# EEA-sensors/parallel-gps

Measured on AMD Instinct MI355X. Metric: timesteps/sec (filter+smooth+log-lik), higher is better.
Workload: dtype f64; 1 GPU; c2: matern32 state-dim 2, N=2^20 steps per GPU (1048576 total), f64, irregular times, prior-sampled observations; steps_per_gpu=1048576, steps_total=1048576, state_dim=2, parallelism=1 GPU

## Files before the change

### parallel-gps_amd/csrc/pgps_ctx.hip

```cpp
#include <cstdio>
#include <new>

#include "pgps_host.h"

using namespace pgps;

namespace pgps {
int ensure(pgps_ctx* ctx, DevBuf& b, size_t bytes) {
    if (&b == &ctx->ws) ++ctx->ws_epoch;
    if (bytes <= b.cap) return PGPS_OK;
    if (b.p) HIPCHK(ctx, hipFree(b.p));
    b.p = nullptr;
    b.cap = 0;
    size_t want = bytes + bytes / 8 + 256;
    hipError_t e = hipMalloc(&b.p, want);
    if (e != hipSuccess) {
        ctx->hip_err = std::string("hipMalloc: ") + hipGetErrorString(e);
        (void)hipGetLastError();
        b.p = nullptr;
        return PGPS_E_NOMEM;
    }
    b.cap = want;
    return PGPS_OK;
}
}

extern "C" int pgps_version(void) { return 100; }

extern "C" const char* pgps_strerror(int code) {
    switch (code) {
        case PGPS_OK: return "ok";
        case PGPS_E_INVALID: return "invalid argument";
        case PGPS_E_UNSUPPORTED_DIM: return "state dimension not supported by the compiled kernels";
        case PGPS_E_HIP: return "HIP runtime error";
        case PGPS_E_NOMEM: return "out of memory";
        case PGPS_E_NUMERIC: return "non-finite result";
        case PGPS_E_NO_DEVICE: return "no HIP device";
        case PGPS_E_COMM: return "RCCL communicator error (pgps_last_hip_error)";
        default: return "unknown error";
    }
}

extern "C" int pgps_device_count(int* n) {
    if (!n) return PGPS_E_INVALID;
    int c = 0;
    if (hipGetDeviceCount(&c) != hipSuccess) c = 0;
    *n = c;
    return PGPS_OK;
}

extern "C" int pgps_create(int device, pgps_ctx** out) {
    if (!out) return PGPS_E_INVALID;
    *out = nullptr;
    int c = 0;
    if (hipGetDeviceCount(&c) != hipSuccess || c <= 0) return PGPS_E_NO_DEVICE;
    if (device < 0 || device >= c) return PGPS_E_INVALID;
    pgps_ctx* ctx = new (std::nothrow) pgps_ctx();
    if (!ctx) return PGPS_E_NOMEM;
    ctx->device = device;
    if (hipSetDevice(device) != hipSuccess ||
        hipStreamCreateWithFlags(&ctx->own_stream, hipStreamNonBlocking) != hipSuccess) {
        delete ctx;
        return PGPS_E_HIP;
    }
    ctx->stream = ctx->own_stream;
    if (hipDeviceGetAttribute(&ctx->n_cu, hipDeviceAttributeMultiprocessorCount, device) != hipSuccess) ctx->n_cu = 0;
    if (const char* e = std::getenv("PGPS_WC_ROWS2")) ctx->wc_rows2 = std::atoi(e) & 15;
    if (const char* e = std::getenv("PGPS_WC_SERIAL3")) ctx->wc_serial3 = (e[0] == '1');
    if (hipMalloc((void**)&ctx->status_word, pgps::kStatusBytes) != hipSuccess ||
        hipMemset(ctx->status_word, 0, pgps::kStatusBytes) != hipSuccess) {
        (void)hipStreamDestroy(ctx->own_stream);
        delete ctx;
        return PGPS_E_NOMEM;
    }
    *out = ctx;
    return PGPS_OK;
}

extern "C" int pgps_destroy(pgps_ctx* ctx) {
    if (!ctx) return PGPS_OK;
    (void)hipSetDevice(ctx->device);
    (void)hipStreamSynchronize(ctx->stream);
    if (ctx->comm) (void)pgps_comm_destroy(ctx);
    if (ctx->comm_buf.p) (void)hipFree(ctx->comm_buf.p);
    if (ctx->ws.p) (void)hipFree(ctx->ws.p);
    if (ctx->stamps.p) (void)hipFree(ctx->stamps.p);
    if (ctx->res_stamps.p) (void)hipFree(ctx->res_stamps.p);
    if (ctx->gadj.p) (void)hipFree(ctx->gadj.p);
    if (ctx->pin_d.p) (void)hipFree(ctx->pin_d.p);
    if (ctx->pin_h) (void)hipHostFree(ctx->pin_h);
    if (ctx->out_h) (void)hipHostFree(ctx->out_h);
    if (ctx->status_word) (void)hipFree(ctx->status_word);
    for (auto& b : ctx->st)
        if (b.p) (void)hipFree(b.p);
    for (auto& b : ctx->lti)
        if (b.p) (void)hipFree(b.p);
    for (auto& b : ctx->wide)
        if (b.p) (void)hipFree(b.p);
    if (ctx->smp.p) (void)hipFree(ctx->smp.p);
    if (ctx->smp_wide.p) (void)hipFree(ctx->smp_wide.p);
    if (ctx->probe_host) (void)hipHostFree(ctx->probe_host);
    for (auto& e : ctx->ev_pool) { (void)hipEventDestroy(e.a); (void)hipEventDestroy(e.b); }
    if (ctx->own_stream) (void)hipStreamDestroy(ctx->own_stream);
    delete ctx;
    return PGPS_OK;
}

extern "C" int pgps_set_stream(pgps_ctx* ctx, void* s) {
    if (!ctx) return PGPS_E_INVALID;
    ctx->stream = (hipStream_t)s;
    return PGPS_OK;
}

extern "C" int pgps_use_own_stream(pgps_ctx* ctx) {
    if (!ctx) return PGPS_E_INVALID;
    ctx->stream = ctx->own_stream;
    return PGPS_OK;
}

extern "C" int pgps_synchronize(pgps_ctx* ctx) {
    if (!ctx) return PGPS_E_INVALID;
    HIPCHK(ctx, hipStreamSynchronize(ctx->stream));
    return PGPS_OK;
}

extern "C" int pgps_set_chunk(pgps_ctx* ctx, int c) {
    if (!ctx || c < 0) return PGPS_E_INVALID;
    ctx->chunk = c;
    return PGPS_OK;
}

extern "C" int pgps_debug_read_stamps(pgps_ctx* ctx, long long* out, long n_values) {
    if (!ctx || !out) return PGPS_E_INVALID;
    if (!ctx->stamps.p || (size_t)n_values * sizeof(long long) > ctx->stamps.cap) return PGPS_E_INVALID;
    HIPCHK(ctx, hipStreamSynchronize(ctx->stream));
    HIPCHK(ctx, hipMemcpy(out, ctx->stamps.p, (size_t)n_values * sizeof(long long), hipMemcpyDeviceToHost));
    return PGPS_OK;
}

extern "C" int pgps_status(pgps_ctx* ctx, int* flags) {
    if (!ctx || !flags) return PGPS_E_INVALID;
    *flags = 0;
    if (!ctx->status_word) return PGPS_OK;
    HIPCHK(ctx, hipStreamSynchronize(ctx->stream));
    HIPCHK(ctx, hipMemcpy(flags, ctx->status_word, sizeof(int), hipMemcpyDeviceToHost));
// ... 372 lines not shown
```

### parallel-gps_amd/csrc/pgps_internal.h

```cpp
#pragma once

#include <hip/hip_runtime.h>
#include <hip/hip_ext.h>

#include <string>
#include <vector>

#include "../../include/pgps.h"
#include "pgps_dyn.h"

struct DevBuf {
    void* p = nullptr;
    size_t cap = 0;
};

struct pgps_ctx {
    int device = 0;
    int n_cu = 0;
    hipStream_t own_stream = nullptr;
    hipStream_t stream = nullptr;
    int chunk = 0;
    int stage_g = -1;
    int single_pass = -1;
    int lookback_window = 256;
    int block = 0;
    size_t batch_scratch = 0;
    int batch_form = 0;
    int one_launch = -1;
    long grad_pack = -1;
    int rc_scan = -1;
    int dma = -1;
    int shortcut = 1;
    int resident = -1;
    unsigned res_epoch = 0;
    DevBuf res_stamps;
    int res_stamp_blocks = 0;
    int res_delay_tile = -1;
    int res_delay_phase = 0;
    long long res_delay_ticks = 0;
    int family = 0;
    std::string hip_err;
    DevBuf ws;
    DevBuf st[12];
    bool wc_attr_done[2][17] = {};
    int wc_rows2 = 15;
    int wc_serial3 = 0;
    DevBuf lti[12];
    DevBuf stamps;
    int* status_word = nullptr;
    int host_flags = 0;
    int f32_policy = 0;
    int* probe_host = nullptr;
    int* probe_dev = nullptr;
    int probe_seq = 0;
    int f32_last_promoted = 0;
    char* pin_h = nullptr;
    DevBuf pin_d;
    char* out_h = nullptr;
    size_t out_cap = 0;
    DevBuf gadj;
    DevBuf wide[9];
    DevBuf smp;
    DevBuf smp_wide;
    DevBuf cov[6];
    DevBuf cov_wide;
    void* comm = nullptr;
    int comm_rank = 0, comm_nranks = 0;
    DevBuf comm_buf;
    struct SegTag { int phase = 0; long N = 0; int d = 0, rank = 0, nranks = 0, chunk = 0, block = 0, family = 0, stage_g = 0, dma = 0, rc_scan = 0; unsigned long epoch = 0; } seg_tag;
    unsigned long ws_epoch = 0;
    unsigned profiling = 0;
    int prof_every = 1;
    long prof_seen[PGPS_K_COUNT] = {0};
    struct EvPair { hipEvent_t a, b; int slot; };
    std::vector<EvPair> ev_pool;
    size_t ev_used = 0;
    double prof_ms[PGPS_K_COUNT] = {0};
    long prof_n[PGPS_K_COUNT] = {0};
};

struct RoctxRange {
    explicit RoctxRange(const char* name) { pgps::dyn::range_push(name); }
    ~RoctxRange() { pgps::dyn::range_pop(); }
    RoctxRange(const RoctxRange&) = delete;
    RoctxRange& operator=(const RoctxRange&) = delete;
};

// ... 57 lines not shown
    int nt;
    int* ticket;
    int* flags;
    int ll_in_apply;
    T* incl;
    int win;
    long long* stamps;
    int shortcut;
    int dform;
};

inline int seg_rec_f_len(int d) { return d * d + d + d * (d + 1) + d + 2 * d * d; }
inline int seg_rec_s_pad(int d) { int n = d * d + d + d * (d + 1) / 2; return n + (n & 1); }
inline int seg_rec_s_len(int d) { return seg_rec_s_pad(d) + 2; }

template <typename... KArgs, typename... Args>
inline void timed_launch(pgps_ctx* ctx, int slot, void (*kernel)(KArgs...), dim3 grid, dim3 block, unsigned shmem,
                         Args... args) {
    pgps_ctx::EvPair* ev = prof_acquire(ctx, slot);
    if (ev) hipExtLaunchKernelGGL(kernel, grid, block, shmem, ctx->stream, ev->a, ev->b, 0, KArgs(args)...);
    else hipLaunchKernelGGL(kernel, grid, block, shmem, ctx->stream, KArgs(args)...);
}

template <typename T>
struct GpModel {
    double lam;
    double N1[9];
    double N2[9];
    double Pinf[9];
    T H[3];
    const T* ts;
    T t_prev;
};

template <typename T>
struct GpArgs {
    ScanArgs<T> s;
    GpModel<T> m;
    const int* qslot;
    T* pmean;
    T* pvar;
};

template <typename T, int D>
int launch_gp(pgps_ctx* ctx, GpArgs<T> g, int want_filtered, int want_smoothed);

template <typename T>
struct ResArgs {
    ScanArgs<T> s;
    GpModel<T> m;
    int* bar;
    int* bar2;
    int* bar_next;
    int* flags1;
    int* flags2;
    int epoch;
    long long* stamps;
    int delay_tile;
    int delay_phase;
    long long delay_ticks;
    long long* wstamps;
};
constexpr int kResLc = 16;
constexpr int kStatusBytes = 8192;
constexpr int kResBarWord = 512;
constexpr int kResBarSet = 2 * 8 * 32;
constexpr int kResFlagWord = 1536;
constexpr int kResMaxBlocks = 256;
static_assert(kResBarWord + 2 * kResBarSet <= kResFlagWord, "barrier counters overlap the hand-off flags");
static_assert((kResFlagWord + 2 * kResMaxBlocks) * 4 <= kStatusBytes, "hand-off flags outside the status buffer");
bool resident_fits(const pgps_ctx* ctx, long N, int d, bool f32);
template <typename T, int D>
int launch_resident(pgps_ctx* ctx, ResArgs<T> ra, bool fused, bool smooth);
template <typename T, int D>
int launch_gp_adj(pgps_ctx* ctx, GpArgs<double> g, double* out);

template <typename T>
struct GpBatchArgs {
    long N;
    int Lc, nblocks;
    long nlanes;
    const T* ts;
    const T* ys;
    T t_prev;
    const double* models;
    T* spine;
    T* lpre;
    double* llpart;
    double* ll;
    T* fms;
    T* fPs;
    long bs_fm, bs_fP;
    T* sspine;
    T* lsuf;
    const int* qslot;
    T* pmean;
    T* pvar;
    long K;
};
constexpr int kGpModelStride = 32;

template <typename T, int D>
int launch_gp_batch(pgps_ctx* ctx, int B, GpBatchArgs<T> b);
template <typename T, int D>
int launch_gp_predict_batch(pgps_ctx* ctx, int B, GpBatchArgs<T> b);
template <typename T, int D>
int launch_gp_adj_batch(pgps_ctx* ctx, int B, GpBatchArgs<double> b, double* out);
constexpr size_t kBatchScratchDefault = 64u << 20;
constexpr long kBatchOneMax = 65536;

template <typename T>
int launch_merge(pgps_ctx* ctx, long N, long K, const T* ts, const T* ys, const T* tq, T* ts_m, T* ys_m, int* qslot);

int launch_grad(pgps_ctx* ctx, long N, int d, int np, const double* model, const double* ts, double t0,
                const double* ys, double* out_dev);

template <int D>
int launch_gradb(pgps_ctx* ctx, long N, int nblk, const int* bsize, int np, const double* model, const double* ts, double t0,
                 const double* ys, double* out_dev);

enum Mode { MODE_PKF, MODE_PKS, MODE_PKFS, MODE_SEG_REDUCE, MODE_SEG_FILTER, MODE_SEG_SMOOTHER };

template <typename T>
// ... 138 lines not shown
```

### parallel-gps_amd/csrc/pgps_res_inst.hip

```cpp
#include "pgps_resident.hip.h"

#ifndef PGPS_RES_T
#error "compile with -DPGPS_RES_T=<float|double> -DPGPS_RES_D=<d>"
#endif

namespace pgps {

template <typename T, int D>
int launch_resident(pgps_ctx* ctx, ResArgs<T> ra, bool fused, bool smooth) {
    HIPCHK(ctx, hipSetDevice(ctx->device));
    ScanArgs<T>& a = ra.s;
    const int max_blocks = ctx->n_cu < kResMaxBlocks ? ctx->n_cu : kResMaxBlocks;
    int lc = kResLc;
    if (ctx->resident > 0 && (ctx->chunk == 8 || ctx->chunk == 16)) lc = ctx->chunk;
    else if (a.N <= (long)kBlock * 8 * max_blocks) lc = 8;
    a.Lc = lc;
    a.nblocks = (int)((a.N + (long)kBlock * lc - 1) / ((long)kBlock * lc));
    if (a.nblocks < 1 || a.nblocks > max_blocks) return PGPS_E_INVALID;
    a.nlanes = (long)a.nblocks * kBlock;
    a.seg_first = 1;
    a.seg_last = 1;
    a.shortcut = ctx->shortcut != 0 ? 1 : 0;
    auto up = [](size_t x) { return (x + 255) / 256 * 256; };
    const size_t nb = (size_t)a.nblocks;
    size_t off = 0;
    const size_t o_spine = off;  off = up(off + nb * Dim<D>::NFILT * sizeof(T));
    const size_t o_sspine = off; off = up(off + nb * Dim<D>::NSMTH * sizeof(T));
    const size_t o_ll = off;     off = up(off + nb * sizeof(double));
    int rc = ensure(ctx, ctx->ws, off);
    if (rc) return rc;
    ctx->ws_epoch++;
    char* base = (char*)ctx->ws.p;
    a.spine = (T*)(base + o_spine);
    a.sspine = (T*)(base + o_sspine);
    a.llpart = (double*)(base + o_ll);
    a.status = ctx->status_word;
    const unsigned e = ctx->res_epoch++;
    ra.bar = ctx->status_word + kResBarWord + (e & 1u) * kResBarSet;
    ra.bar2 = ra.bar + kResBarSet / 2;
    ra.bar_next = ctx->status_word + kResBarWord + ((e + 1u) & 1u) * kResBarSet;
    ra.flags1 = ctx->status_word + kResFlagWord;
    ra.flags2 = ctx->status_word + kResFlagWord + kResMaxBlocks;
    ra.epoch = (int)(e % 0x7ffffffeu) + 1;
    ra.stamps = nullptr;
    ra.wstamps = nullptr;
    ra.delay_tile = -1;
    ra.delay_phase = 0;
    ra.delay_ticks = 0;
    const bool skew = ctx->res_delay_tile >= 0;
    if (ctx->resident == 2 || skew) {
        rc = ensure(ctx, ctx->res_stamps, nb * (16 + 8) * sizeof(long long));
        if (rc) return rc;
        if (ctx->resident == 2) ra.stamps = (long long*)ctx->res_stamps.p;
        ctx->res_stamp_blocks = a.nblocks;
    }
    if (skew) {
        HIPCHK(ctx, hipMemsetAsync(ctx->res_stamps.p, 0, nb * 16 * sizeof(long long), ctx->stream));
        HIPCHK(ctx, hipMemsetAsync(base, 0xFF, off, ctx->stream));
        ra.wstamps = (long long*)ctx->res_stamps.p;
        ra.delay_tile = ctx->res_delay_tile;
        ra.delay_phase = ctx->res_delay_phase;
        ra.delay_ticks = ctx->res_delay_ticks;
    }
    const dim3 grid(a.nblocks), block(kBlock);
    auto go = [&](auto lcv, auto fusedv, auto smoothv) {
        constexpr int L = decltype(lcv)::value;
        constexpr bool FU = decltype(fusedv)::value, SM = decltype(smoothv)::value;
        if (skew) timed_launch(ctx, PGPS_K_RESIDENT, k_pkfs_resident<T, D, L, FU, SM, true>, grid, block, 0, ra);
        else timed_launch(ctx, PGPS_K_RESIDENT, k_pkfs_resident<T, D, L, FU, SM, false>, grid, block, 0, ra);
    };
    auto pick = [&](auto lcv) {
        if (fused) { if (smooth) go(lcv, std::true_type{}, std::true_type{}); else go(lcv, std::true_type{}, std::false_type{}); }
        else { if (smooth) go(lcv, std::false_type{}, std::true_type{}); else go(lcv, std::false_type{}, std::false_type{}); }
    };
    if (lc == 8) pick(std::integral_constant<int, 8>{}); else pick(std::integral_constant<int, kResLc>{});
    HIPCHK(ctx, hipGetLastError());
    return PGPS_OK;
}

template int launch_resident<PGPS_RES_T, PGPS_RES_D>(pgps_ctx*, ResArgs<PGPS_RES_T>, bool, bool);

}
```

### parallel-gps_amd/csrc/pgps_resident.hip.h

```cpp
#pragma once

#include <type_traits>

#include "pgps_fused.hip.h"
#include "pgps_kernels.hip.h"

namespace pgps {


template <typename T, int D, int LC>
struct ResCfg {
    static constexpr int W = (int)sizeof(T), MAT = D * D, G = 4;
    static_assert(LC % G == 0, "whole sub-tiles");
    static constexpr int S = LC / G;
    using GF = StageGeom<MAT * W, G>;
    using GM = StageGeom<D * W, G>;
    static constexpr int SLOT = LC * MAT * W + 16;
    static constexpr int SLOTS = kWave * SLOT;
    static constexpr int MST = GM::BYTES > 5120 ? GM::BYTES : 5120;
    static constexpr int NSCAN = kWaves * Dim<D>::NFILT * W;
    static constexpr int BYTES = kWaves * (SLOTS + MST) + NSCAN + kWaves * 8;
};

__device__ __forceinline__ void res_wave_sync() {
    __builtin_amdgcn_fence(__ATOMIC_RELEASE, "wavefront");
    __builtin_amdgcn_wave_barrier();
    __builtin_amdgcn_fence(__ATOMIC_ACQUIRE, "wavefront");
}

template <typename T> struct ResForget;
template <> struct ResForget<double> { static constexpr double kA = 0x1p-120; };
template <> struct ResForget<float> { static constexpr float kA = 0x1p-60f; };

#define PGPS_RSTAMP(IDX)                                                                              \
    do {                                                                                              \
        if (ra.stamps && threadIdx.x == 0) ra.stamps[(long)blockIdx.x * 16 + (IDX)] = __builtin_readcyclecounter(); \
    } while (0)
#define PGPS_RSTAMP_WAVE(K)                                                                           \
    do {                                                                                              \
        if (ra.stamps && lane == 0)                                                                   \
            ra.stamps[(long)gridDim.x * 16 + (long)blockIdx.x * 8 + (K) * kWaves + wave] = __builtin_readcyclecounter(); \
    } while (0)

template <typename T>
__device__ __forceinline__ void res_skew(const ResArgs<T>& ra, int tile, int phase) {
    if (tile == ra.delay_tile && phase == ra.delay_phase) {
        const long long t0 = wall_clock64();
        ra.wstamps[(long)tile * 16 + 12] = t0;
        ra.wstamps[(long)tile * 16 + 13] = ra.delay_ticks;
        while (wall_clock64() - t0 < ra.delay_ticks) __builtin_amdgcn_s_sleep(8);
    }
}
template <typename T>
__device__ __forceinline__ void res_wstamp(const ResArgs<T>& ra, int tile, int slot) {
    if (ra.wstamps) ra.wstamps[(long)tile * 16 + slot] = wall_clock64();
}

template <typename T, int D>
__device__ __forceinline__ V4 res_pad_piece(int kind, int pos_in_rec) {
    constexpr int PER = 16 / (int)sizeof(T);
    T tmp[PER];
#pragma unroll
    for (int j = 0; j < PER; ++j) {
        const int e = (pos_in_rec * PER + j) % (D * D);
        tmp[j] = (kind == 0 && (e / D) == (e % D)) ? T(1) : T(0);
    }
    V4 v;
    __builtin_memcpy(&v, tmp, 16);
    return v;
}

template <typename T, int D, typename GEO, int PITCH>
__device__ __forceinline__ void res_issue(const char* __restrict__ g , int sb, long lim, bool full, int kind, V4* r) {
// ... 34 lines not shown
#pragma unroll
        for (int v = 0; v < NV; ++v)
            if (v >= v0 && v < v0 + nv) x[v] = *reinterpret_cast<const V4*>(base + sb * GEO::SEG + v * OPI * SLOT);
#pragma unroll
        for (int v = 0; v < NV; ++v)
            if (v >= v0 && v < v0 + nv) *reinterpret_cast<V4*>(g + ((long)sb * GEO::SEG + (long)v * OPI * PITCH) + loff) = x[v];
    } else {
#pragma unroll
        for (int v = 0; v < NV; ++v) {
            if (v < v0 || v >= v0 + nv) continue;
            const V4 x = *reinterpret_cast<const V4*>(base + sb * GEO::SEG + v * OPI * SLOT);
            if ((int)loff < lim - (sb * GEO::SEG + v * OPI * PITCH))
                *reinterpret_cast<V4*>(g + ((long)sb * GEO::SEG + (long)v * OPI * PITCH) + loff) = x;
        }
    }
}
template <typename GEO, int SLOT, int PITCH>
__device__ __forceinline__ void res_drain(char* __restrict__ g , int sb, int lim, bool full, const char* slots) {
    res_drain_part<GEO, SLOT, PITCH>(g, sb, 0, GEO::NV, lim, full, slots);
}
template <typename GEO, int PITCH>
__device__ __forceinline__ void res_drain_m(char* __restrict__ g , int sb, int lim, bool full, const char* mst) {
    const int lane = threadIdx.x & (kWave - 1);
    constexpr int NV = GEO::NV, OPI = kWave / NV;
    const char* base = mst + (lane / NV) * GEO::STRIDE + (lane % NV) * 16;
    const unsigned loff = (unsigned)(lane / NV) * PITCH + (unsigned)(lane % NV) * 16u;
    if (full) {
        V4 x[NV];
#pragma unroll
        for (int v = 0; v < NV; ++v) x[v] = *reinterpret_cast<const V4*>(base + v * OPI * GEO::STRIDE);
#pragma unroll
        for (int v = 0; v < NV; ++v) *reinterpret_cast<V4*>(g + ((long)sb * GEO::SEG + (long)v * OPI * PITCH) + loff) = x[v];
    } else {
#pragma unroll
        for (int v = 0; v < NV; ++v) {
            const V4 x = *reinterpret_cast<const V4*>(base + v * OPI * GEO::STRIDE);
            if ((int)loff < lim - (sb * GEO::SEG + v * OPI * PITCH))
                *reinterpret_cast<V4*>(g + ((long)sb * GEO::SEG + (long)v * OPI * PITCH) + loff) = x;
        }
    }
}

__device__ __forceinline__ void res_wait_all(int* bar, int nblocks, int* status) {
    if (threadIdx.x < 8) {
        const int want = (nblocks - (int)threadIdx.x + 7) / 8;
        if (want > 0) wait_flag(bar + threadIdx.x * 32, want, status);
    }
    __syncthreads();
}
__device__ __forceinline__ void res_arrive(int* bar, int tile) {
    __hip_atomic_fetch_add(bar + (tile & 7) * 32, 1, __ATOMIC_RELAXED, __HIP_MEMORY_SCOPE_AGENT);
}

__device__ __forceinline__ bool res_wait_epoch(const int* f, int want, int* status) {
    int spins = 0;
    while (__hip_atomic_load(f, __ATOMIC_RELAXED, __HIP_MEMORY_SCOPE_AGENT) != want) {
        __builtin_amdgcn_s_sleep(2);
        if (++spins > (1 << 22)) {
            atomicOr(status, 2);
            return false;
        }
    }
    return true;
}

template <typename T, int D>
__device__ __forceinline__ void res_filt_extend(FiltElem<T, D>& e, const T* F, const T* Q , T y, const T* h, T R) {
    T Ap[D * D], bp[D], FC[D * D], Cp[Dim<D>::SYM];
    mat_mul<T, D>(F, e.A, Ap);
    mat_vec<T, D>(F, e.b, bp);
    predict_cov<T, D>(F, e.C, Q, FC, Cp);
    const bool obs = !is_nan(y);
    T u[D], v[D];
    sym_vec<T, D>(Cp, h, u);
    mat_t_vec<T, D>(Ap, h, v);
    T S = R, hb = T(0);
#pragma unroll
    for (int i = 0; i < D; ++i) { S += h[i] * u[i]; hb += h[i] * bp[i]; }
    const T inv = obs ? recip(S) : T(0);
    const T res = obs ? y - hb : T(0);
#pragma unroll
    for (int i = 0; i < D; ++i) {
        const T Ki = u[i] * inv;
#pragma unroll
        for (int j = 0; j < D; ++j) e.A[i * D + j] = Ap[i * D + j] - Ki * v[j];
        e.b[i] = bp[i] + Ki * res;
        e.eta[i] += v[i] * (res * inv);
    }
#pragma unroll
    for (int i = 0; i < D; ++i)
#pragma unroll
        for (int j = i; j < D; ++j) {
            e.C[symi<D>(i, j)] = Cp[symi<D>(i, j)] - u[i] * u[j] * inv;
            e.J[symi<D>(i, j)] += v[i] * v[j] * inv;
        }
}

template <typename T, int D>
__device__ __forceinline__ void res_kf_step(MeanCov<T, D>& s, const T* F, const T* Q , T y, const T* h, T R, LogLik& ll,
                                            T* mp, T* Pp, T* FP) {
    mat_vec<T, D>(F, s.m, mp);
    predict_cov<T, D>(F, s.P, Q, FP, Pp);
    const bool obs = !is_nan(y);
    T u[D];
    sym_vec<T, D>(Pp, h, u);
    T S = R, mu = T(0);
#pragma unroll
    for (int i = 0; i < D; ++i) { S += h[i] * u[i]; mu += h[i] * mp[i]; }
    const T rinv = recip(S);
    {
        const double r = obs ? ll_diff(y, mu) : 0.0;
        const double Sw = obs ? ll_wide(S) : 1.0;
        ll.quad += r * r * (obs ? double(rinv) : 0.0);
        int e;
        ll.mant = std::frexp(ll.mant * Sw, &e);
        ll.expo += e;
// ... 91 lines not shown
    if constexpr (FORWARD) {
        all(res_dpp_elem<kDppRowShr + 1>(incl, r >= 1));
        all(res_dpp_elem<kDppRowShr + 2>(incl, r >= 2));
        all(res_dpp_elem<kDppRowShr + 4>(incl, r >= 4));
        all(res_dpp_elem<kDppRowShr + 8>(incl, r >= 8));
        step(dpp_elem<kDppBcast15, 0xa>(incl), (lane & 16) != 0);
        step(dpp_elem<kDppBcast31, 0xc>(incl), lane >= 32);
    } else {
        all(res_dpp_elem<kDppRowShl + 1>(incl, r + 1 < 16));
        all(res_dpp_elem<kDppRowShl + 2>(incl, r + 2 < 16));
        all(res_dpp_elem<kDppRowShl + 4>(incl, r + 4 < 16));
        all(res_dpp_elem<kDppRowShl + 8>(incl, r + 8 < 16));
        const int row = lane >> 4;
        step(shfl_idx_elem(incl, ((row + 1) & 3) * 16), row < 3);
        step(shfl_idx_elem(incl, ((row + 2) & 3) * 16), row < 2);
    }
#else
    wave_scan_inclusive<E, FORWARD>(incl, lane);
#endif
}

template <typename E, bool FORWARD>
__device__ __forceinline__ void res_scan4(E& x, int lane) {
    using TR = ElemTraits<E>;
    const int r = lane & 15;
    auto all = [&](const E& other) {
        E t;
        if (FORWARD) TR::combine(other, x, t); else TR::combine(x, other, t);
        x = t;
    };
    if constexpr (FORWARD) {
        all(res_dpp_elem<kDppRowShr + 1>(x, r >= 1));
        all(res_dpp_elem<kDppRowShr + 2>(x, r >= 2));
    } else {
        all(res_dpp_elem<kDppRowShl + 1>(x, r + 1 < 16));
        all(res_dpp_elem<kDppRowShl + 2>(x, r + 2 < 16));
    }
}
template <typename E, bool FORWARD, typename PUB>
__device__ __forceinline__ void res_block_scan_exclusive(const E& mine, E& excl, typename ElemTraits<E>::Scalar* lds, PUB&& publish) {
    using TR = ElemTraits<E>;
    static_assert(kWaves == 4, "four wave totals in lanes 0..3");
    const int lane = threadIdx.x & (kWave - 1);
    const int wave = __builtin_amdgcn_readfirstlane((int)(threadIdx.x / kWave));
    E incl = mine;
    res_wave_scan_inclusive<E, FORWARD>(incl, lane);
    E wex = FORWARD ? res_dpp_elem<kDppWaveShr1>(incl, lane != 0) : res_dpp_elem<kDppWaveShl1>(incl, lane != kWave - 1);
    if (FORWARD ? (lane == kWave - 1) : (lane == 0)) rec_store(lds + wave * TR::N, incl);
    __syncthreads();
    E t;
    TR::identity(t);
    if (lane < kWaves) rec_load(lds + lane * TR::N, t);
    res_scan4<E, FORWARD>(t, lane);
    if (threadIdx.x == (FORWARD ? kWaves - 1 : 0)) publish(t);
    typename TR::Scalar pv[TR::N], iv[TR::N];
    {
        E id;
        TR::identity(id);
        pack(id, iv);
        pack(t, pv);
    }
    const bool edge = FORWARD ? (wave == 0) : (wave == kWaves - 1);
    const int src = FORWARD ? (edge ? 0 : wave - 1) : (edge ? 0 : wave + 1);
#pragma unroll
    for (int i = 0; i < TR::N; ++i) { const typename TR::Scalar x = res_readlane(pv[i], src); pv[i] = edge ? iv[i] : x; }
    E p;
    unpack(pv, p);
    if (FORWARD) TR::combine(p, wex, excl); else TR::combine(wex, p, excl);
    __syncthreads();
}
template <typename E>
__device__ __forceinline__ void res_block_reduce_ordered(const E& mine, E& total, typename ElemTraits<E>::Scalar* lds) {
    using TR = ElemTraits<E>;
    const int lane = threadIdx.x & (kWave - 1);
    const int wave = __builtin_amdgcn_readfirstlane((int)(threadIdx.x / kWave));
    E acc = mine;
    res_wave_scan_inclusive<E, true>(acc, lane);
    if (lane == kWave - 1) rec_store(lds + wave * TR::N, acc);
    __syncthreads();
    E t;
    TR::identity(t);
    if (lane < kWaves) rec_load(lds + lane * TR::N, t);
    res_scan4<E, true>(t, lane);
    total = res_readlane_elem(t, kWaves - 1);
    __syncthreads();
}

template <typename T, int LC>
struct ResLaneValues {
    using GY = StageGeom<64, 1>;
    static constexpr int PER = 64 / (int)sizeof(T);
    static constexpr int R = LC / PER > 0 ? LC / PER : 1;
    static_assert(LC % PER == 0, "whole rounds");
    V4 r[R][GY::NV];
    __device__ __forceinline__ void issue(const T* __restrict__ g ) {
        const int lane = threadIdx.x & (kWave - 1);
        constexpr int NV = GY::NV, OPI = kWave / NV, PITCH = LC * (int)sizeof(T);
        const unsigned loff = (unsigned)(lane / NV) * PITCH + (unsigned)(lane % NV) * 16u;
#pragma unroll
        for (int rd = 0; rd < R; ++rd)
#pragma unroll
            for (int v = 0; v < NV; ++v)
                r[rd][v] = *reinterpret_cast<const V4*>(reinterpret_cast<const char*>(g) + ((long)rd * 64 + (long)v * OPI * PITCH) + loff);
    }
    __device__ __forceinline__ void finish(char* mst, T* out) {
        const int lane = threadIdx.x & (kWave - 1);
#pragma unroll
        for (int rd = 0; rd < R; ++rd) {
            res_wave_sync();
            constexpr int NV = GY::NV, OPI = kWave / NV;
            char* base = mst + (lane / NV) * GY::STRIDE + (lane % NV) * 16;
#pragma unroll
            for (int v = 0; v < NV; ++v) *reinterpret_cast<V4*>(base + v * OPI * GY::STRIDE) = r[rd][v];
            res_wave_sync();
            load_rec<T, PER>(reinterpret_cast<const T*>(mst + lane * GY::STRIDE), out + rd * PER);
        }
        res_wave_sync();
    }
};

template <typename T, int D, int LC, bool FUSED, bool SMOOTH = true, bool SKEW = false>
__global__ __launch_bounds__(kBlock) void k_pkfs_resident(const ResArgs<T> ra) {
    using CFG = ResCfg<T, D, LC>;
    using GF = typename CFG::GF;
    using GM = typename CFG::GM;
    using FE = FiltElem<T, D>;
    using SE = SmthElem<T, D>;
    using MC = MeanCov<T, D>;
    constexpr int MAT = D * D, SYM = Dim<D>::SYM, NF = Dim<D>::NFILT, NS = Dim<D>::NSMTH, G = CFG::G, S = CFG::S;
    constexpr int SLOT = CFG::SLOT;
    static_assert(kBlock == 256, "one workgroup of four waves per CU");
    static_assert(D <= 2, "resident pass: d <= 2");
    const ScanArgs<T>& a = ra.s;

    __shared__ __attribute__((aligned(16))) char smem[CFG::BYTES];
    const int tile = blockIdx.x;
    const int lane = threadIdx.x & (kWave - 1);
    const int wave = __builtin_amdgcn_readfirstlane((int)(threadIdx.x / kWave));
    char* slots = smem + wave * CFG::SLOTS;
    char* mst = smem + kWaves * CFG::SLOTS + wave * CFG::MST;
    T* lds = reinterpret_cast<T*>(smem + kWaves * (CFG::SLOTS + CFG::MST));
    double* lds_ll = reinterpret_cast<double*>(smem + kWaves * (CFG::SLOTS + CFG::MST) + CFG::NSCAN);
    char* myslot = slots + lane * SLOT;
    T* myrec = reinterpret_cast<T*>(myslot);

    PGPS_RSTAMP(0);
    if (tile == 0 && threadIdx.x < 16) ra.bar_next[threadIdx.x * 32] = 0;

    const long N = a.N;
    const long gt = (long)tile * kBlock + threadIdx.x;
    const long k0 = gt * LC;
    const long wbase = ((long)tile * kBlock + wave * kWave) * LC;
    const bool full = (wbase + (long)kWave * LC <= N);
    constexpr int PF = LC * MAT * (int)sizeof(T), PM = LC * D * (int)sizeof(T);
    const long limF = (N - wbase) * MAT * (long)sizeof(T);
    const int limP = res_lim32(limF), limM = res_lim32((N - wbase) * D * (long)sizeof(T));

    T h[D], P0[SYM];
    if constexpr (FUSED) {
        gp_prior<T, D>(ra.m, h, P0);
    } else {
        T P0f[MAT];
#pragma unroll
        for (int i = 0; i < MAT; ++i) P0f[i] = a.P0[i];
        sym_from_full<T, D>(P0f, P0);
#pragma unroll
        for (int i = 0; i < D; ++i) h[i] = a.H[i];
    }
    const T Rn = a.R;

    T Freg[LC][MAT];
    T yreg[LC];
    constexpr int GL = MAT - SYM;
    static_assert(D - GL == 1, "one component of g per step stays in registers");
    FE agg;
    filt_identity(agg);
    auto reduce_step = [&](int j, const T* Qf) {
        T Q[SYM];
        sym_from_full<T, D>(Qf, Q);
        if (j == 0) {
            if (k0 == 0) filt_first(agg, P0, yreg[0], h, Rn);
            else res_filt_extend(agg, Freg[0], Q, yreg[0], h, Rn);
        } else {
            res_filt_extend(agg, Freg[j], Q, yreg[j], h, Rn);
        }
    };
    {
        const T nanv = T(__builtin_nan(""));
        if constexpr (FUSED) {
            T tv[LC];
            const T* tp = ra.m.ts;
            T tprev;
            if (full) {
                ResLaneValues<T, LC> lt, ly;
// ... 23 lines not shown
            }
        } else {
            const char* gF = reinterpret_cast<const char*>(a.Fs + wbase * MAT);
            const char* gQ = reinterpret_cast<const char*>(a.Qs + wbase * MAT);
            auto stream = [&](auto full_tag) {
                constexpr bool FULL = decltype(full_tag)::value;
                V4 rF[2][GF::NV], rQ[2][GF::NV];
                ResLaneValues<T, LC> ly;
                if constexpr (FULL) ly.issue(a.ys + wbase);
                res_issue<T, D, GF, PF>(gF, 0, limF, FULL, 0, rF[0]);
                res_issue<T, D, GF, PF>(gQ, 0, limF, FULL, 1, rQ[0]);
                if (S > 1) {
                    res_issue<T, D, GF, PF>(gF, 1, limF, FULL, 0, rF[1]);
                    res_issue<T, D, GF, PF>(gQ, 1, limF, FULL, 1, rQ[1]);
                }
                if constexpr (FULL) {
                    ly.finish(mst, yreg);
                } else {
#pragma unroll
                    for (int j = 0; j < LC; ++j) yreg[j] = (k0 + j < N) ? a.ys[k0 + j < N ? k0 + j : 0] : nanv;
                }
#pragma unroll
                for (int sb = 0; sb < S; ++sb) {
                    const int p = sb & 1;
                    res_wave_sync();
                    res_commit<GF, SLOT>(slots, sb, rF[p]);
                    if (sb + 2 < S) res_issue<T, D, GF, PF>(gF, sb + 2, limF, FULL, 0, rF[p]);
                    res_wave_sync();
#pragma unroll
                    for (int i = 0; i < G; ++i) load_rec<T, MAT>(myrec + (sb * G + i) * MAT, Freg[sb * G + i]);
                    res_wave_sync();
                    res_commit<GF, SLOT>(slots, sb, rQ[p]);
                    if (sb + 2 < S) res_issue<T, D, GF, PF>(gQ, sb + 2, limF, FULL, 1, rQ[p]);
                    res_wave_sync();
#pragma unroll
                    for (int i = 0; i < G; ++i) {
                        const int j = sb * G + i;
                        T Qf[MAT];
                        load_rec<T, MAT>(myrec + j * MAT, Qf);
                        reduce_step(j, Qf);
                        __builtin_amdgcn_sched_barrier(0);
                    }
                }
            };
            if (full) stream(std::true_type{}); else stream(std::false_type{});
        }
    }
    PGPS_RSTAMP_WAVE(0);
    PGPS_RSTAMP(1);
    FE excl;
    res_block_scan_exclusive<FE, true>(agg, excl, lds, [&](const FE& total) {
        T v[NF];
        pack(total, v);
        if constexpr (SKEW) res_skew(ra, tile, 1);
#pragma unroll
        for (int i = 0; i < NF; ++i) pub_store(a.spine + (long)tile * NF + i, v[i]);
        asm volatile("s_waitcnt vmcnt(0)" ::: "memory");
        pub_store(ra.flags1 + tile, ra.epoch);
        if constexpr (SKEW) res_wstamp(ra, tile, 10);
        res_arrive(ra.bar, tile);
    });
    PGPS_RSTAMP(2);

    MC s;
#pragma unroll
    for (int i = 0; i < D; ++i) s.m[i] = T(0);
#pragma unroll
    for (int i = 0; i < SYM; ++i) s.P[i] = P0[i];
    bool waited_all = false;
    if (tile > 0) {
        if (a.shortcut != 0) {
            if (threadIdx.x == 0) res_wait_epoch(ra.flags1 + tile - 1, ra.epoch, a.status);
            __syncthreads();
        } else {
            res_wait_all(ra.bar, a.nblocks, a.status);
            waited_all = true;
        }
        FE nb;
        {
            T v[NF];
#pragma unroll
            for (int i = 0; i < NF; ++i) v[i] = pub_load(a.spine + (long)(tile - 1) * NF + i);
            unpack(v, nb);
        }
        T amax = T(0);
#pragma unroll
        for (int i = 0; i < MAT; ++i) amax = fmax(amax, fabs(nb.A[i]));
        const bool forget = a.shortcut != 0 && amax <= ResForget<T>::kA;
        if (__builtin_amdgcn_readfirstlane((int)forget)) {
#pragma unroll
            for (int i = 0; i < D; ++i) s.m[i] = nb.b[i];
#pragma unroll
            for (int i = 0; i < SYM; ++i) s.P[i] = nb.C[i];
        } else {
            if (!waited_all) res_wait_all(ra.bar, a.nblocks, a.status);
            FE mine, left;
            filt_identity(mine);
            if ((int)threadIdx.x < tile) {
                T v[NF];
                const T* rec = reinterpret_cast<const T*>(reinterpret_cast<const char*>(a.spine) + threadIdx.x * (unsigned)(NF * sizeof(T)));
#pragma unroll
                for (int i = 0; i < NF; ++i) v[i] = pub_load(rec + i);
                unpack(v, mine);
            }
            res_block_reduce_ordered(mine, left, lds);
            filt_apply(s, left);
        }
    }
    PGPS_RSTAMP(3);
    filt_apply(s, excl);
    PGPS_RSTAMP(4);

    LogLik ll;
    SE sagg;
    smth_identity(sagg);
    T Fh[MAT], Qh[MAT];
    T Qn[MAT];
    load_rec<T, MAT>(myrec, Qn);
    if constexpr (SMOOTH) {
#pragma unroll
        for (int i = 0; i < MAT; ++i) {
            Fh[i] = wshfl_down(Freg[0][i], 1);
            Qh[i] = wshfl_down(Qn[i], 1);
        }
        if (lane == kWave - 1) {
            const long k1 = k0 + LC;
            if (k1 < N) {
                if constexpr (FUSED) {
                    lti_step<T, D>(ra.m, ra.m.ts[k1] - ra.m.ts[k1 - 1], Fh, Qh);
                } else {
                    load_rec<T, MAT>(a.Fs + k1 * MAT, Fh);
                    load_rec<T, MAT>(a.Qs + k1 * MAT, Qh);
                }
            } else {
#pragma unroll
                for (int i = 0; i < MAT; ++i) { Fh[i] = (i / D == i % D) ? T(1) : T(0); Qh[i] = T(0); }
            }
        }
    }
    const int to_end = (N - k0 < 0) ? -1 : (N - k0 > LC ? LC + 1 : (int)(N - k0));
    auto element = [&](int j_next, const MC& prev, const T* mp, const T* Pp, T* FP, SE& e) {
        const bool last = (j_next == to_end);
#pragma unroll
        for (int q = 0; q < MAT; ++q) FP[q] = last ? T(0) : FP[q];
        smth_element(prev, mp, Pp, FP, e);
    };
    const bool store_f = (a.fms != nullptr);
    char* gP = reinterpret_cast<char*>(a.fPs + wbase * MAT);
    char* gM = reinterpret_cast<char*>(a.fms + wbase * D);
    constexpr int NVP = GF::NV, PPS = (NVP + G - 2) / (G - 1);
    T Lhold[MAT];
    T Lwait[G - 1][MAT];
#pragma unroll
    for (int sb = 0; sb < S; ++sb) {
        T Lnew[G - 1][MAT];
// ... 58 lines not shown
        PGPS_RSTAMP_WAVE(1);
        PGPS_RSTAMP(5);
        const double v = ll.value();
        const double t = block_sum_double(v, lds_ll);
        if (threadIdx.x == 0) {
            if constexpr (SKEW) res_skew(ra, tile, 2);
            pub_store(a.llpart + tile, t);
            asm volatile("s_waitcnt vmcnt(0)" ::: "memory");
            if constexpr (SKEW) res_wstamp(ra, tile, 11);
            res_arrive(ra.bar2, tile);
        }
        if (tile == 0 && a.ll != nullptr) {
            res_wait_all(ra.bar2, a.nblocks, a.status);
            double w = 0.0;
            for (int b = threadIdx.x; b < a.nblocks; b += kBlock) w += pub_load(a.llpart + b);
            const double tt = block_sum_double(w, lds_ll);
            if (threadIdx.x == 0) *a.ll = tt;
        }
        PGPS_RSTAMP(9);
        return;
    }
    {
        if (store_f) res_drain_part<GF, SLOT, PF>(gP, S - 1, 0, NVP / 2, limP, full, slots);
        constexpr int j = LC - 1;
        T Q[SYM], mp[D], Pp[SYM], FP[MAT];
        sym_from_full<T, D>(Qh, Q);
        mat_vec<T, D>(Fh, s.m, mp);
        predict_cov<T, D>(Fh, s.P, Q, FP, Pp);
        SE e, r;
        element(LC, s, mp, Pp, FP, e);
        smth_combine(sagg, e, r);
        sagg = r;
#pragma unroll
        for (int q = 0; q < MAT; ++q) Freg[j][q] = e.E[q];
        yreg[j] = e.g[D - 1];
        T Lg[MAT];
#pragma unroll
        for (int q = 0; q < MAT; ++q) Lg[q] = q < SYM ? e.L[q < SYM ? q : 0] : e.g[q < SYM ? 0 : q - SYM];
#pragma unroll
        for (int q = 0; q < MAT; ++q) asm volatile("" : "+v"(Lg[q]));
        __builtin_amdgcn_sched_barrier(0);
        if (store_f) res_drain_part<GF, SLOT, PF>(gP, S - 1, NVP / 2, NVP - NVP / 2, limP, full, slots);
        res_wave_sync();
#pragma unroll
        for (int i = 0; i + 1 < G; ++i) store_rec<T, MAT>(myrec + ((S - 1) * G + i) * MAT, Lwait[i]);
        store_rec<T, MAT>(myrec + j * MAT, Lg);
    }
    PGPS_RSTAMP_WAVE(1);
    PGPS_RSTAMP(5);
    SE sexcl;
    res_block_scan_exclusive<SE, false>(sagg, sexcl, lds, [&](const SE& stotal) {
        T vv[NS];
        pack(stotal, vv);
        if constexpr (SKEW) res_skew(ra, tile, 2);
#pragma unroll
        for (int i = 0; i < NS; ++i) pub_store(a.sspine + (long)tile * NS + i, vv[i]);
        asm volatile("s_waitcnt vmcnt(0)" ::: "memory");
        pub_store(ra.flags2 + tile, ra.epoch);
    });
    PGPS_RSTAMP(6);
    {
        const double v = ll.value();
        const double t = block_sum_double(v, lds_ll);
        if (threadIdx.x == 0) {
            pub_store(a.llpart + tile, t);
            asm volatile("s_waitcnt vmcnt(0)" ::: "memory");
            if constexpr (SKEW) res_wstamp(ra, tile, 11);
            res_arrive(ra.bar2, tile);
        }
    }

#pragma unroll
    for (int i = 0; i < D; ++i) s.m[i] = T(0);
#pragma unroll
    for (int i = 0; i < SYM; ++i) s.P[i] = T(0);
    waited_all = false;
    if (tile + 1 < a.nblocks) {
        if (a.shortcut != 0) {
            if (threadIdx.x == 0) res_wait_epoch(ra.flags2 + tile + 1, ra.epoch, a.status);
            __syncthreads();
        } else {
            res_wait_all(ra.bar2, a.nblocks, a.status);
            waited_all = true;
        }
        SE nb;
        {
            T v[NS];
#pragma unroll
            for (int i = 0; i < NS; ++i) v[i] = pub_load(a.sspine + (long)(tile + 1) * NS + i);
            unpack(v, nb);
        }
        T emax = T(0);
#pragma unroll
        for (int i = 0; i < MAT; ++i) emax = fmax(emax, fabs(nb.E[i]));
        const bool forget = a.shortcut != 0 && emax <= ResForget<T>::kA;
        if (__builtin_amdgcn_readfirstlane((int)forget)) {
#pragma unroll
            for (int i = 0; i < D; ++i) s.m[i] = nb.g[i];
#pragma unroll
            for (int i = 0; i < SYM; ++i) s.P[i] = nb.L[i];
        } else {
            if (!waited_all) { res_wait_all(ra.bar2, a.nblocks, a.status); waited_all = true; }
            SE mine, right;
            smth_identity(mine);
            const int b = tile + 1 + (int)threadIdx.x;
            if (b < a.nblocks) {
                T v[NS];
                const T* rec = reinterpret_cast<const T*>(reinterpret_cast<const char*>(a.sspine + (long)(tile + 1) * NS) +
                                                          threadIdx.x * (unsigned)(NS * sizeof(T)));
#pragma unroll
                for (int i = 0; i < NS; ++i) v[i] = pub_load(rec + i);
                unpack(v, mine);
            }
            res_block_reduce_ordered(mine, right, lds);
            smth_apply(right, s);
        }
    }
    PGPS_RSTAMP(7);
    smth_apply(sexcl, s);
    PGPS_RSTAMP(8);
    if (tile == 0 && a.ll != nullptr) {
        if (!waited_all) res_wait_all(ra.bar2, a.nblocks, a.status);
        double v = 0.0;
        for (int b = threadIdx.x; b < a.nblocks; b += kBlock) v += pub_load(a.llpart + b);
        const double t = block_sum_double(v, lds_ll);
        if (threadIdx.x == 0) *a.ll = t;
    }
    char* oP = reinterpret_cast<char*>(a.sPs + wbase * MAT);
    char* oM = reinterpret_cast<char*>(a.sms + wbase * D);
    T Ln[MAT];
    load_rec<T, MAT>(myrec + (LC - 1) * MAT, Ln);
#pragma unroll
    for (int sb = S - 1; sb >= 0; --sb) {
#pragma unroll
        for (int i = G - 1; i >= 0; --i) {
            const int j = sb * G + i;
            SE e;
#pragma unroll
            for (int q = 0; q < MAT; ++q) e.E[q] = Freg[j][q];
            e.g[D - 1] = yreg[j];
#pragma unroll
            for (int q = 0; q < SYM; ++q) e.L[q] = Ln[q];
#pragma unroll
            for (int q = SYM; q < MAT; ++q) e.g[q - SYM] = Ln[q];
            if (j > 0) load_rec<T, MAT>(myrec + (j - 1) * MAT, Ln);
            smth_apply(e, s);
            T Pf[MAT];
            full_from_sym<T, D>(s.P, Pf);
            store_rec<T, MAT>(myrec + j * MAT, Pf);
            store_rec<T, D>(reinterpret_cast<T*>(mst + lane * GM::STRIDE) + i * D, s.m);
        }
        res_wave_sync();
        res_drain<GF, SLOT, PF>(oP, sb, limP, full, slots);
        res_drain_m<GM, PM>(oM, sb, limM, full, mst);
        res_wave_sync();
    }
    PGPS_RSTAMP(9);
}

}
```

Baseline: 23.41 billion timesteps/s.

## Publish block-scan carries as epoch-tagged 64-bit words instead of data-plus-flag

Replaces the spine arrays plus separate epoch flags in the resident kernel with per-tile records in which each 32-bit payload word is packed with the epoch into one 64-bit atomic store. A consumer polls all words of the record at once and is done when every word carries the current epoch. This removes the store-fence-flag sequence on the producer and the extra flag round trip on the consumer. The first poll of the right neighbour's smoothing record is also issued early, before the log-likelihood reduction. In exchange each record takes one 256-byte slot per tile in a new buffer, the publish goes through LDS with a wave sync, and the slow path now reads records word by word.

Measured after the change: 23.87 billion timesteps/s, median of 6. 1.02x the previous value.

```diff
diff --git a/parallel-gps_amd/csrc/pgps_ctx.hip b/parallel-gps_amd/csrc/pgps_ctx.hip
--- a/parallel-gps_amd/csrc/pgps_ctx.hip
+++ b/parallel-gps_amd/csrc/pgps_ctx.hip
@@ -68,7 +68,11 @@
     if (const char* e = std::getenv("PGPS_WC_ROWS2")) ctx->wc_rows2 = std::atoi(e) & 15;
     if (const char* e = std::getenv("PGPS_WC_SERIAL3")) ctx->wc_serial3 = (e[0] == '1');
     if (hipMalloc((void**)&ctx->status_word, pgps::kStatusBytes) != hipSuccess ||
-        hipMemset(ctx->status_word, 0, pgps::kStatusBytes) != hipSuccess) {
+        hipMemset(ctx->status_word, 0, pgps::kStatusBytes) != hipSuccess ||
+        hipMalloc((void**)&ctx->res_gran, pgps::kResGranBytes) != hipSuccess ||
+        hipMemset(ctx->res_gran, 0, pgps::kResGranBytes) != hipSuccess) {
+        if (ctx->res_gran) (void)hipFree(ctx->res_gran);
+        if (ctx->status_word) (void)hipFree(ctx->status_word);
         (void)hipStreamDestroy(ctx->own_stream);
         delete ctx;
         return PGPS_E_NOMEM;
@@ -91,6 +95,7 @@
     if (ctx->pin_h) (void)hipHostFree(ctx->pin_h);
     if (ctx->out_h) (void)hipHostFree(ctx->out_h);
     if (ctx->status_word) (void)hipFree(ctx->status_word);
+    if (ctx->res_gran) (void)hipFree(ctx->res_gran);
     for (auto& b : ctx->st)
         if (b.p) (void)hipFree(b.p);
     for (auto& b : ctx->lti)
diff --git a/parallel-gps_amd/csrc/pgps_internal.h b/parallel-gps_amd/csrc/pgps_internal.h
--- a/parallel-gps_amd/csrc/pgps_internal.h
+++ b/parallel-gps_amd/csrc/pgps_internal.h
@@ -33,6 +33,7 @@
     int shortcut = 1;
     int resident = -1;
     unsigned res_epoch = 0;
+    unsigned long long* res_gran = nullptr;
     DevBuf res_stamps;
     int res_stamp_blocks = 0;
     int res_delay_tile = -1;
@@ -196,8 +197,8 @@
     int* bar;
     int* bar2;
     int* bar_next;
-    int* flags1;
-    int* flags2;
+    unsigned long long* gran1;
+    unsigned long long* gran2;
     int epoch;
     long long* stamps;
     int delay_tile;
@@ -209,10 +210,10 @@
 constexpr int kStatusBytes = 8192;
 constexpr int kResBarWord = 512;
 constexpr int kResBarSet = 2 * 8 * 32;
-constexpr int kResFlagWord = 1536;
 constexpr int kResMaxBlocks = 256;
-static_assert(kResBarWord + 2 * kResBarSet <= kResFlagWord, "barrier counters overlap the hand-off flags");
-static_assert((kResFlagWord + 2 * kResMaxBlocks) * 4 <= kStatusBytes, "hand-off flags outside the status buffer");
+static_assert((kResBarWord + 2 * kResBarSet) * 4 <= kStatusBytes, "barrier counters outside the status buffer");
+constexpr int kResGranStride = 256;
+constexpr size_t kResGranBytes = 2 * (size_t)kResMaxBlocks * kResGranStride;
 bool resident_fits(const pgps_ctx* ctx, long N, int d, bool f32);
 template <typename T, int D>
 int launch_resident(pgps_ctx* ctx, ResArgs<T> ra, bool fused, bool smooth);
diff --git a/parallel-gps_amd/csrc/pgps_res_inst.hip b/parallel-gps_amd/csrc/pgps_res_inst.hip
--- a/parallel-gps_amd/csrc/pgps_res_inst.hip
+++ b/parallel-gps_amd/csrc/pgps_res_inst.hip
@@ -23,24 +23,21 @@
     a.shortcut = ctx->shortcut != 0 ? 1 : 0;
     auto up = [](size_t x) { return (x + 255) / 256 * 256; };
     const size_t nb = (size_t)a.nblocks;
-    size_t off = 0;
-    const size_t o_spine = off;  off = up(off + nb * Dim<D>::NFILT * sizeof(T));
-    const size_t o_sspine = off; off = up(off + nb * Dim<D>::NSMTH * sizeof(T));
-    const size_t o_ll = off;     off = up(off + nb * sizeof(double));
+    const size_t off = up(nb * sizeof(double));
     int rc = ensure(ctx, ctx->ws, off);
     if (rc) return rc;
     ctx->ws_epoch++;
     char* base = (char*)ctx->ws.p;
-    a.spine = (T*)(base + o_spine);
-    a.sspine = (T*)(base + o_sspine);
-    a.llpart = (double*)(base + o_ll);
+    a.spine = nullptr;
+    a.sspine = nullptr;
+    a.llpart = (double*)base;
     a.status = ctx->status_word;
     const unsigned e = ctx->res_epoch++;
     ra.bar = ctx->status_word + kResBarWord + (e & 1u) * kResBarSet;
     ra.bar2 = ra.bar + kResBarSet / 2;
     ra.bar_next = ctx->status_word + kResBarWord + ((e + 1u) & 1u) * kResBarSet;
-    ra.flags1 = ctx->status_word + kResFlagWord;
-    ra.flags2 = ctx->status_word + kResFlagWord + kResMaxBlocks;
+    ra.gran1 = ctx->res_gran;
+    ra.gran2 = ctx->res_gran + (size_t)kResMaxBlocks * kResGranStride / sizeof(unsigned long long);
     ra.epoch = (int)(e % 0x7ffffffeu) + 1;
     ra.stamps = nullptr;
     ra.wstamps = nullptr;
@@ -57,6 +54,7 @@
     if (skew) {
         HIPCHK(ctx, hipMemsetAsync(ctx->res_stamps.p, 0, nb * 16 * sizeof(long long), ctx->stream));
         HIPCHK(ctx, hipMemsetAsync(base, 0xFF, off, ctx->stream));
+        HIPCHK(ctx, hipMemsetAsync(ctx->res_gran, 0xFF, kResGranBytes, ctx->stream));
         ra.wstamps = (long long*)ctx->res_stamps.p;
         ra.delay_tile = ctx->res_delay_tile;
         ra.delay_phase = ctx->res_delay_phase;
diff --git a/parallel-gps_amd/csrc/pgps_resident.hip.h b/parallel-gps_amd/csrc/pgps_resident.hip.h
--- a/parallel-gps_amd/csrc/pgps_resident.hip.h
+++ b/parallel-gps_amd/csrc/pgps_resident.hip.h
@@ -18,7 +18,9 @@
     static constexpr int SLOT = LC * MAT * W + 16;
     static constexpr int SLOTS = kWave * SLOT;
     static constexpr int MST = GM::BYTES > 5120 ? GM::BYTES : 5120;
-    static constexpr int NSCAN = kWaves * Dim<D>::NFILT * W;
+    static constexpr int NREC = Dim<D>::NFILT * W;
+    static constexpr int NSCAN = (kWaves + 1) * NREC;
+    static_assert(NSCAN % 8 == 0, "the log-likelihood sum's doubles follow the scan scratch");
     static constexpr int BYTES = kWaves * (SLOTS + MST) + NSCAN + kWaves * 8;
 };
 
@@ -159,16 +161,64 @@
     __hip_atomic_fetch_add(bar + (tile & 7) * 32, 1, __ATOMIC_RELAXED, __HIP_MEMORY_SCOPE_AGENT);
 }
 
-__device__ __forceinline__ bool res_wait_epoch(const int* f, int want, int* status) {
-    int spins = 0;
-    while (__hip_atomic_load(f, __ATOMIC_RELAXED, __HIP_MEMORY_SCOPE_AGENT) != want) {
-        __builtin_amdgcn_s_sleep(2);
-        if (++spins > (1 << 22)) {
-            atomicOr(status, 2);
-            return false;
-        }
-    }
-    return true;
+template <typename T, int N>
+struct ResGran {
+    static constexpr int WPS = (int)sizeof(T) / 4;
+    static constexpr int NG = N * WPS;
+    static_assert(NG <= kWave && NG * 8 <= kResGranStride, "one wave-instruction and one place per record");
+};
+__device__ __forceinline__ unsigned long long* res_gran_rec(unsigned long long* g, int tile) {
+    return g + (long)tile * (kResGranStride / 8);
+}
+template <typename T, int N>
+__device__ __forceinline__ void res_publish(unsigned long long* rec, unsigned* hand, const T* v, int holder, int epoch) {
+    constexpr int NG = ResGran<T, N>::NG;
+    const int lane = threadIdx.x & (kWave - 1);
+    if (lane == holder) {
+        unsigned w[NG];
+        __builtin_memcpy(w, v, sizeof(w));
+#pragma unroll
+        for (int i = 0; i < NG; ++i) hand[i] = w[i];
+    }
+    res_wave_sync();
+    if (lane < NG) {
+        const unsigned long long x = ((unsigned long long)(unsigned)epoch << 32) | hand[lane];
+        __hip_atomic_store(rec + lane, x, __ATOMIC_RELAXED, __HIP_MEMORY_SCOPE_AGENT);
+    }
+}
+template <typename T, int N>
+__device__ __forceinline__ unsigned long long res_poll_first(const unsigned long long* rec) {
+    if (threadIdx.x < ResGran<T, N>::NG) return __hip_atomic_load(rec + threadIdx.x, __ATOMIC_RELAXED, __HIP_MEMORY_SCOPE_AGENT);
+    return 0ull;
+}
+template <typename T, int N>
+__device__ __forceinline__ void res_take(const unsigned long long* rec, unsigned long long x, int epoch, unsigned* hand, int* status, T* v) {
+    constexpr int NG = ResGran<T, N>::NG;
+    if (__builtin_amdgcn_readfirstlane((int)threadIdx.x) == 0) {
+        const bool polls = threadIdx.x < NG;
+        bool stale = polls && (unsigned)(x >> 32) != (unsigned)epoch;
+        int spins = 0;
+        while (__builtin_amdgcn_ballot_w64(stale) != 0 && ++spins <= (1 << 22)) {
+            __builtin_amdgcn_s_sleep(2);
+            if (polls) x = __hip_atomic_load(rec + threadIdx.x, __ATOMIC_RELAXED, __HIP_MEMORY_SCOPE_AGENT);
+            stale = polls && (unsigned)(x >> 32) != (unsigned)epoch;
+        }
+        if (stale) atomicOr(status, 2);
+        if (polls) hand[threadIdx.x] = (unsigned)x;
+    }
+    __syncthreads();
+    unsigned w[NG];
+#pragma unroll
+    for (int i = 0; i < NG; ++i) w[i] = hand[i];
+    __builtin_memcpy(v, w, sizeof(w));
+}
+template <typename T, int N>
+__device__ __forceinline__ void res_load_record(const unsigned long long* rec, T* v) {
+    constexpr int NG = ResGran<T, N>::NG;
+    unsigned w[NG];
+#pragma unroll
+    for (int i = 0; i < NG; ++i) w[i] = (unsigned)__hip_atomic_load(rec + i, __ATOMIC_RELAXED, __HIP_MEMORY_SCOPE_AGENT);
+    __builtin_memcpy(v, w, sizeof(w));
 }
 
 template <typename T, int D>
@@ -366,7 +416,7 @@
     TR::identity(t);
     if (lane < kWaves) rec_load(lds + lane * TR::N, t);
     res_scan4<E, FORWARD>(t, lane);
-    if (threadIdx.x == (FORWARD ? kWaves - 1 : 0)) publish(t);
+    if (wave == 0) publish(t);
     typename TR::Scalar pv[TR::N], iv[TR::N];
     {
         E id;
@@ -454,6 +504,7 @@
     char* slots = smem + wave * CFG::SLOTS;
     char* mst = smem + kWaves * CFG::SLOTS + wave * CFG::MST;
     T* lds = reinterpret_cast<T*>(smem + kWaves * (CFG::SLOTS + CFG::MST));
+    unsigned* hand = reinterpret_cast<unsigned*>(smem + kWaves * (CFG::SLOTS + CFG::MST) + kWaves * CFG::NREC);
     double* lds_ll = reinterpret_cast<double*>(smem + kWaves * (CFG::SLOTS + CFG::MST) + CFG::NSCAN);
     char* myslot = slots + lane * SLOT;
     T* myrec = reinterpret_cast<T*>(myslot);
@@ -583,14 +634,16 @@
     res_block_scan_exclusive<FE, true>(agg, excl, lds, [&](const FE& total) {
         T v[NF];
         pack(total, v);
-        if constexpr (SKEW) res_skew(ra, tile, 1);
-#pragma unroll
-        for (int i = 0; i < NF; ++i) pub_store(a.spine + (long)tile * NF + i, v[i]);
+        if constexpr (SKEW) { if (lane == kWaves - 1) res_skew(ra, tile, 1); }
+        res_publish<T, NF>(res_gran_rec(ra.gran1, tile), hand, v, kWaves - 1, ra.epoch);
+    });
+    if (wave == 0) {
         asm volatile("s_waitcnt vmcnt(0)" ::: "memory");
-        pub_store(ra.flags1 + tile, ra.epoch);
-        if constexpr (SKEW) res_wstamp(ra, tile, 10);
-        res_arrive(ra.bar, tile);
-    });
+        if (lane == 0) {
+            if constexpr (SKEW) res_wstamp(ra, tile, 10);
+            res_arrive(ra.bar, tile);
+        }
+    }
     PGPS_RSTAMP(2);
 
     MC s;
@@ -598,40 +651,31 @@
     for (int i = 0; i < D; ++i) s.m[i] = T(0);
 #pragma unroll
     for (int i = 0; i < SYM; ++i) s.P[i] = P0[i];
-    bool waited_all = false;
     if (tile > 0) {
+        FE nb;
+        bool forget = false;
         if (a.shortcut != 0) {
-            if (threadIdx.x == 0) res_wait_epoch(ra.flags1 + tile - 1, ra.epoch, a.status);
-            __syncthreads();
+            const unsigned long long* rec = res_gran_rec(ra.gran1, tile - 1);
+            T v[NF];
+            res_take<T, NF>(rec, res_poll_first<T, NF>(rec), ra.epoch, hand, a.status, v);
+            unpack(v, nb);
+            T amax = T(0);
+#pragma unroll
+            for (int i = 0; i < MAT; ++i) amax = fmax(amax, fabs(nb.A[i]));
+            forget = amax <= ResForget<T>::kA;
+        }
+        if (__builtin_amdgcn_readfirstlane((int)forget)) {
+#pragma unroll
+            for (int i = 0; i < D; ++i) s.m[i] = nb.b[i];
+#pragma unroll
+            for (int i = 0; i < SYM; ++i) s.P[i] = nb.C[i];
         } else {
             res_wait_all(ra.bar, a.nblocks, a.status);
-            waited_all = true;
-        }
-        FE nb;
-        {
-            T v[NF];
-#pragma unroll
-            for (int i = 0; i < NF; ++i) v[i] = pub_load(a.spine + (long)(tile - 1) * NF + i);
-            unpack(v, nb);
-        }
-        T amax = T(0);
-#pragma unroll
-        for (int i = 0; i < MAT; ++i) amax = fmax(amax, fabs(nb.A[i]));
-        const bool forget = a.shortcut != 0 && amax <= ResForget<T>::kA;
-        if (__builtin_amdgcn_readfirstlane((int)forget)) {
-#pragma unroll
-            for (int i = 0; i < D; ++i) s.m[i] = nb.b[i];
-#pragma unroll
-            for (int i = 0; i < SYM; ++i) s.P[i] = nb.C[i];
-        } else {
-            if (!waited_all) res_wait_all(ra.bar, a.nblocks, a.status);
             FE mine, left;
             filt_identity(mine);
             if ((int)threadIdx.x < tile) {
                 T v[NF];
-                const T* rec = reinterpret_cast<const T*>(reinterpret_cast<const char*>(a.spine) + threadIdx.x * (unsigned)(NF * sizeof(T)));
-#pragma unroll
-                for (int i = 0; i < NF; ++i) v[i] = pub_load(rec + i);
+                res_load_record<T, NF>(res_gran_rec(ra.gran1, (int)threadIdx.x), v);
                 unpack(v, mine);
             }
             res_block_reduce_ordered(mine, left, lds);
@@ -796,13 +840,13 @@
     res_block_scan_exclusive<SE, false>(sagg, sexcl, lds, [&](const SE& stotal) {
         T vv[NS];
         pack(stotal, vv);
-        if constexpr (SKEW) res_skew(ra, tile, 2);
-#pragma unroll
-        for (int i = 0; i < NS; ++i) pub_store(a.sspine + (long)tile * NS + i, vv[i]);
-        asm volatile("s_waitcnt vmcnt(0)" ::: "memory");
-        pub_store(ra.flags2 + tile, ra.epoch);
+        if constexpr (SKEW) { if (lane == 0) res_skew(ra, tile, 2); }
+        res_publish<T, NS>(res_gran_rec(ra.gran2, tile), hand, vv, 0, ra.epoch);
     });
     PGPS_RSTAMP(6);
+    const bool take_right = tile + 1 < a.nblocks && a.shortcut != 0;
+    unsigned long long poll0 = 0ull;
+    if (take_right) poll0 = res_poll_first<T, NS>(res_gran_rec(ra.gran2, tile + 1));
     {
         const double v = ll.value();
         const double t = block_sum_double(v, lds_ll);
@@ -818,42 +862,33 @@
     for (int i = 0; i < D; ++i) s.m[i] = T(0);
 #pragma unroll
     for (int i = 0; i < SYM; ++i) s.P[i] = T(0);
-    waited_all = false;
+    bool waited_all = false;
     if (tile + 1 < a.nblocks) {
-        if (a.shortcut != 0) {
-            if (threadIdx.x == 0) res_wait_epoch(ra.flags2 + tile + 1, ra.epoch, a.status);
-            __syncthreads();
+        SE nb;
+        bool forget = false;
+        if (take_right) {
+            T v[NS];
+            res_take<T, NS>(res_gran_rec(ra.gran2, tile + 1), poll0, ra.epoch, hand, a.status, v);
+            unpack(v, nb);
+            T emax = T(0);
+#pragma unroll
+            for (int i = 0; i < MAT; ++i) emax = fmax(emax, fabs(nb.E[i]));
+            forget = emax <= ResForget<T>::kA;
+        }
+        if (__builtin_amdgcn_readfirstlane((int)forget)) {
+#pragma unroll
+            for (int i = 0; i < D; ++i) s.m[i] = nb.g[i];
+#pragma unroll
+            for (int i = 0; i < SYM; ++i) s.P[i] = nb.L[i];
         } else {
             res_wait_all(ra.bar2, a.nblocks, a.status);
             waited_all = true;
-        }
-        SE nb;
-        {
-            T v[NS];
-#pragma unroll
-            for (int i = 0; i < NS; ++i) v[i] = pub_load(a.sspine + (long)(tile + 1) * NS + i);
-            unpack(v, nb);
-        }
-        T emax = T(0);
-#pragma unroll
-        for (int i = 0; i < MAT; ++i) emax = fmax(emax, fabs(nb.E[i]));
-        const bool forget = a.shortcut != 0 && emax <= ResForget<T>::kA;
-        if (__builtin_amdgcn_readfirstlane((int)forget)) {
-#pragma unroll
-            for (int i = 0; i < D; ++i) s.m[i] = nb.g[i];
-#pragma unroll
-            for (int i = 0; i < SYM; ++i) s.P[i] = nb.L[i];
-        } else {
-            if (!waited_all) { res_wait_all(ra.bar2, a.nblocks, a.status); waited_all = true; }
             SE mine, right;
             smth_identity(mine);
             const int b = tile + 1 + (int)threadIdx.x;
             if (b < a.nblocks) {
                 T v[NS];
-                const T* rec = reinterpret_cast<const T*>(reinterpret_cast<const char*>(a.sspine + (long)(tile + 1) * NS) +
-                                                          threadIdx.x * (unsigned)(NS * sizeof(T)));
-#pragma unroll
-                for (int i = 0; i < NS; ++i) v[i] = pub_load(rec + i);
+                res_load_record<T, NS>(res_gran_rec(ra.gran2, b), v);
                 unpack(v, mine);
             }
             res_block_reduce_ordered(mine, right, lds);
```
